# TheShadow29/VidSitu

Hardware: AMD Instinct MI355X
Metric: clips/s (10s@32x224x224) SlowFast+TxEnc fwd+bwd (higher is better)
Workload: dtype bf16

## Files before the change

include/vidsitu_hip.h:

```cpp
#ifndef VIDSITU_HIP_H
#define VIDSITU_HIP_H

#include <stddef.h>
#include <stdint.h>

#ifdef __cplusplus
extern "C" {
#endif

typedef enum vs_status {
  VS_OK = 0,
  VS_ERR_BAD_ARG = -1,
  VS_ERR_UNSUPPORTED = -2,
  VS_ERR_WORKSPACE = -3,
  VS_ERR_LAUNCH = -4
} vs_status;

#define VS_CONV_AFFINE 1
#define VS_CONV_RESIDUAL 2
#define VS_CONV_RELU 4
#define VS_CONV_STATS 8
#define VS_CONV_NAIVE 16
#define VS_CONV_TILE(id) (((id) + 1) << 8)
#define VS_CONV_RING(ns) (((ns) & 7) << 16)
// ... 88 lines not shown
                     const vs_dgrad_epilogue* ep, void* workspace, size_t ws_bytes, void* stream);
int vs_weight_transpose(const void* w, void* wt, int Cout, int taps, int Cin, void* stream);
int vs_weight_transpose_batched(const void* src, void* dst, const int64_t* table, int n,
                                int64_t total, void* stream);
int vs_transpose_f32_batched(const float* src, float* dst, const int64_t* table, int n, int64_t total,
                             void* stream);
int vs_weight_transpose_tiled(const void* src, void* dst, const int64_t* table, const int64_t* tile_first,
                              int n, int64_t total_tiles, int elem_bytes, void* stream);

#define VS_WGRAD_NODEEP (1 << 12)
#define VS_WGRAD_FORCEDEEP (1 << 13)
size_t vs_conv_wgrad_workspace_bytes(const vs_conv_desc* d);
int vs_conv_wgrad(const void* dy, const void* x, float* dw, const vs_conv_desc* d,
                  void* workspace, size_t ws_bytes, void* stream);
typedef struct vs_wgrad_item {
  const void* dy;
  const void* x;
  float* dw;
  vs_conv_desc d;
} vs_wgrad_item;
int vs_conv_wgrad_group_ok(const vs_wgrad_item* items, int n);
size_t vs_conv_wgrad_group_workspace_bytes(const vs_wgrad_item* items, int n);
int vs_conv_wgrad_group(const vs_wgrad_item* items, int n, void* workspace, size_t ws_bytes, void* stream);
int vs_conv_wgrad_partial(const void* dy, const void* x, float* dw, const vs_conv_desc* d, void* slabs,
                          size_t slab_bytes, int* splits, void* stream);
int64_t vs_wgrad_reduce_blocks(int64_t elements);
int vs_wgrad_reduce(const float* slabs, float* dw, int64_t elements, int splits, void* stream);
int vs_wgrad_reduce_batched(const int64_t* table, int n_entries, int64_t total_blocks, void* stream);
int vs_wgrad_reduce_defer(int mode);
int vs_wgrad_reduce_flush(void);

int vs_bn_finalize(const float* partials, int nparts, double count, const float* gamma,
                   const float* beta, float* running_mean, float* running_var, float momentum,
                   float eps, float* scale, float* shift, float* mean, float* invstd, int C,
                   void* stream);
size_t vs_bn_finalize_workspace_bytes(void);
int vs_bn_finalize_ws(const float* partials, int nparts, double count, const float* gamma, const float* beta,
                      float* running_mean, float* running_var, float momentum, float eps, float* scale,
                      float* shift, float* mean, float* invstd, int C, void* workspace, size_t ws_bytes,
                      void* stream);
int vs_bn_partials_reduce(const float* partials, int nparts, float* out, int C, int G,
                          void* stream);
int vs_bn_apply(const void* y, const float* scale, const float* shift, const void* residual,
                void* out, int64_t rows, int C, int y_ld, int res_ld, int out_ld, int relu,
                void* stream);
int vs_bn_apply_mask(const void* y, const float* scale, const float* shift, const void* residual,
// ... 180 lines not shown
```

vidsitu_amd/_lib.py:

```python
import ctypes as C
import os
import subprocess

_HERE = os.path.dirname(os.path.abspath(__file__))
LIB_PATH = os.environ.get("VS_LIB_PATH") or os.path.join(_HERE, "libvidsitu_hip.so")
CSRC_DIR = os.path.join(_HERE, "csrc")

VS_CONV_AFFINE = 1
VS_CONV_RESIDUAL = 2
VS_CONV_RELU = 4
VS_CONV_STATS = 8
VS_CONV_NAIVE = 16


class ConvDesc(C.Structure):

    _fields_ = [
        (n, C.c_int32)
        for n in (
            "N Ti Hi Wi Cin To Ho Wo Cout kT kH kW sT sH sW pT pH pW x_ld y_ld res_ld flags"
        ).split()
    ]


# ... 27 lines not shown
    "vs_conv_fwd": (_i, [_p, _p, _p, _dp, _p, _p, _p, _p, _p, _sz, _p]),
    "vs_conv_stats_rows": (_i, [_dp]),
    "vs_conv_workspace_bytes": (_sz, [_dp, _i]),
    "vs_conv_plan": (_i, [_dp, _i, _p]),
    "vs_conv_aol_ok": (_i, [_dp]),
    "vs_conv_fwd_aol": (_i, [_p, _p, _p, _dp, _p, _p, _p, _p]),
    "vs_conv_wgrad_aol_ok": (_i, [_dp]),
    "vs_conv_wgrad_aol": (_i, [_p, _p, _p, _dp, _p, _p, _p, _sz, _p]),
    "vs_conv_fwd_bc_fusable": (_i, [_dp, _i]),
    "vs_conv_fwd_bc": (_i, [_p, _p, _dp, _p, _p, _p, _i, _p, _p, _p, _i, _p, _i, _i, _p]),
    "vs_conv_dgrad": (_i, [_p, _p, _p, _dp, _p, _p, _sz, _p]),
    "vs_conv_dgrad_bnstats_rows": (_i, [_dp]),
    "vs_conv_dgrad_bnstats": (_i, [_p, _p, _p, _dp, _p, _p, _i, _p, _p, _p, _p, _p, _p, _p, _sz, _p]),
    "vs_conv_dgrad_ex": (_i, [_p, _p, _p, _dp, C.POINTER(DgradEpilogue), _p, _sz, _p]),
    "vs_weight_transpose": (_i, [_p, _p, _i, _i, _i, _p]),
    "vs_weight_transpose_batched": (_i, [_p, _p, _p, _i, _i64, _p]),
    "vs_transpose_f32_batched": (_i, [_p, _p, _p, _i, _i64, _p]),
    "vs_weight_transpose_tiled": (_i, [_p, _p, _p, _p, _i, _i64, _i, _p]),
    "vs_conv_wgrad_workspace_bytes": (_sz, [_dp]),
    "vs_conv_wgrad": (_i, [_p, _p, _p, _dp, _p, _sz, _p]),
    "vs_conv_wgrad_group_ok": (_i, [C.POINTER(WgradItem), _i]),
    "vs_conv_wgrad_group_workspace_bytes": (_sz, [C.POINTER(WgradItem), _i]),
    "vs_conv_wgrad_group": (_i, [C.POINTER(WgradItem), _i, _p, _sz, _p]),
    "vs_conv_wgrad_partial": (_i, [_p, _p, _p, _dp, _p, _sz, C.POINTER(C.c_int), _p]),
    "vs_wgrad_reduce_blocks": (_i64, [_i64]),
    "vs_wgrad_reduce": (_i, [_p, _p, _i64, _i, _p]),
    "vs_wgrad_reduce_batched": (_i, [_p, _i, _i64, _p]),
    "vs_wgrad_reduce_defer": (_i, [_i]),
    "vs_wgrad_reduce_flush": (_i, []),
    "vs_bn_finalize": (_i, [_p, _i, _d, _p, _p, _p, _p, _f, _f, _p, _p, _p, _p, _i, _p]),
    "vs_bn_finalize_workspace_bytes": (_sz, []),
    "vs_bn_finalize_ws": (_i, [_p, _i, _d, _p, _p, _p, _p, _f, _f, _p, _p, _p, _p, _i, _p, _sz, _p]),
    "vs_bn_bwd_finalize_ws": (_i, [_p, _i, _p, _p, _i, _p, _sz, _p]),
    "vs_bn_partials_reduce": (_i, [_p, _i, _p, _i, _i, _p]),
    "vs_bn_apply": (_i, [_p, _p, _p, _p, _p, _i64, _i, _i, _i, _i, _i, _p]),
    "vs_bn_apply_mask": (_i, [_p, _p, _p, _p, _p, _p, _i64, _i, _i, _i, _i, _p]),
    "vs_bn_apply2": (_i, [_p, _p, _p, _p, _p, _p, _p, _p, _i64, _i, _i, _i, _i, _p]),
    "vs_bn_bwd_reduce": (_i, [_p, _p, _p, _p, _p, _p, _p, _p, _i64, _i, _i, _i, _i, _i, _p]),
    "vs_bn_bwd_reduce_rows": (_i, [_i64, _i]),
    "vs_bn_bwd_finalize": (_i, [_p, _i, _p, _p, _i, _p]),
    "vs_bn_bwd_apply": (
        _i,
        [_p, _p, _p, _p, _p, _p, _p, _p, _p, _p, _p, _i64, _i, _i, _i, _i, _i, _i, _i, _p],
    ),
    "vs_bn_bwd_apply2": (_i, [_p] * 16 + [_i64, _i, _i, _i, _i, _i, _i, _p]),
    "vs_residual_add_f32": (_i, [_p, _p, _p, _p, _p, _i64, _i, _i, _i, _i, _i, _i, _p]),
# ... 121 lines not shown
```

vidsitu_amd/csrc/conv_wgrad.hip:

```cpp
#include <stdlib.h>

#include "common.h"

#include <mutex>
#include <type_traits>
#include "glue_bodies.h"

typedef __attribute__((ext_vector_type(4))) short s16x4;
typedef __attribute__((address_space(3))) s16x4 lds_s16x4;

struct WgradP {
  const uint16_t* dy;
  const uint16_t* x;
  float* out;
  int P;
  int Cout, Kp, Cin, x_ld, dy_ld;
  int To, Ho, Wo, Ti, Hi, Wi;
  int kT, kH, kW, sT, sH, sW, pT, pH, pW;
  int tilesM, tilesN, S, rows_per_split;
  unsigned x_bytes, dy_bytes;
  int xcd_order;
  int dbg;
  const float* in_scale;
  const float* in_shift;
};

#define WG_OOB 0x80000000u

#define WG_ROWTAB 1024

__device__ __forceinline__ int wg_swz_chunk(int row) {
  return ((row & 3) << 1) | (((row >> 3) & 1) << 3);
}

template <int BM, int BN, int WM, int WN, int MODE>
__global__ __launch_bounds__(256) void conv_wgrad_kernel(WgradP p) {
  extern __shared__ __attribute__((aligned(16))) char smem[];
  constexpr int TM = BM / WM, TN = BN / WN;
  constexpr int MR = TM / 16, NR = TN / 16;
  constexpr int CM = BM / 8, CN = BN / 8;
  constexpr int RPM = 256 / CM, RPN = 256 / CN;
  constexpr int IM = (64 + RPM - 1) / RPM, IN = (64 + RPN - 1) / RPN;
  constexpr int IMG = 64 * 256;
  constexpr int STAGE = 2 * IMG;
  static_assert(WM * WN == 4, "4 waves");

  const int tid = threadIdx.x;
  int bid = blockIdx.x;
  if (p.xcd_order) {
    const int nwg = gridDim.x, q = nwg >> 3, r = nwg & 7, xcd = blockIdx.x & 7;
    bid = (xcd < r ? xcd * (q + 1) : r * (q + 1) + (xcd - r) * q) + (blockIdx.x >> 3);
  }
  const int ntile = p.tilesM * p.tilesN;
  const int s = bid / ntile;
  bid -= s * ntile;
  const int tn = bid % p.tilesN, tm = bid / p.tilesN;
  const int m0 = tm * BM, n0 = tn * BN;
  const int pbeg = s * p.rows_per_split;
  const int pend = min(p.P, pbeg + p.rows_per_split);

  int4* rowtab = (int4*)(smem + 2 * STAGE);

  const int ccm = tid % CM, rm = tid / CM;
  const int ccn = tid % CN, rn = tid / CN;
  const bool mcol_ok = (m0 + ccm * 8) < p.Cout;
  const int ncol = n0 + ccn * 8;
  const bool ncol_ok = ncol < p.Kp;
  int dt = 0, dh = 0, dw = 0, c0 = 0;
  if (MODE == 1 && ncol_ok) {
    const int tap = ncol / p.Cin;
    c0 = ncol - tap * p.Cin;
    dw = tap % p.kW;
    const int t2 = tap / p.kW;
    dh = t2 % p.kH;
// ... 137 lines not shown
      gload(chunk0 + (st + 1) * 64, chunk0);
      __builtin_amdgcn_sched_barrier(0);
      compute(cur);
      __builtin_amdgcn_sched_barrier(0);
      sstore(cur ^ 1);
      __syncthreads();
    }
    compute((nsteps - 1) & 1);
    __syncthreads();
  }

  float* dst = p.out + (long long)s * p.Cout * p.Kp;
#pragma unroll
  for (int a = 0; a < MR; ++a)
#pragma unroll
    for (int b = 0; b < NR; ++b) {
      const int col = n0 + wn * TN + b * 16 + li;
#pragma unroll
      for (int r = 0; r < 4; ++r) {
        const int row = m0 + wm * TM + a * 16 + g * 4 + r;
        if (row < p.Cout && col < p.Kp) dst[(long long)row * p.Kp + col] = acc[a][b][r];
      }
    }
}

template <int BM, int BN, int WM, int WN, int MODE, int NS, bool AOL = false, int ROWS = 64>
__device__ __forceinline__ void conv_wgrad_ring_body(const WgradP& p, const int blk, const int nblk) {
  static_assert(!AOL || MODE == 0, "apply on load: pointwise launches");
  static_assert(ROWS == 64, "stage depth (the half-depth variant of round 4 was measured slower and removed)");
  extern __shared__ __attribute__((aligned(16))) char smem[];
  constexpr int TM = BM / WM, TN = BN / WN;
  constexpr int MR = TM / 16, NR = TN / 16;
  constexpr int CM = BM / 8, CN = BN / 8;
  constexpr int IMG = ROWS * 256;
  constexpr int STAGE = 2 * IMG;
  constexpr int D = NS - 1;
  constexpr int RG = ROWS / 16;
  constexpr int L = 2 * RG;
  constexpr int SPC = WG_ROWTAB / ROWS;
  static_assert(WM * WN == 4, "4 waves");
  static_assert((D - 1) * L <= 63, "vmcnt range");

  const int tid = threadIdx.x;
  int bid = blk;
  if (p.xcd_order) {
    const int nwg = nblk, q = nwg >> 3, r = nwg & 7, xcd = blk & 7;
// ... 504 lines not shown
  if (g.mode[j] == 0) conv_wgrad_deep_body<0, true>(g.p[j], b - lo, cnt);
  else conv_wgrad_deep_body<1, true>(g.p[j], b - lo, cnt);
}

struct WgReduceGroupP {
  int n;
  long long first[WGG_MAX + 1];
  const float* slabs[WGG_MAX];
  float* dw[WGG_MAX];
  long long len[WGG_MAX];
  int S[WGG_MAX];
};

__global__ __launch_bounds__(256) void wgrad_reduce_group_kernel(WgReduceGroupP g) {
  __shared__ float4 part[16][17];
  const long long b = blockIdx.x;
  int e = 0;
#pragma unroll
  for (int i = 1; i < WGG_MAX; ++i)
    if (i < g.n && b >= g.first[i]) e = i;
  wgrad_reduce_body(g.slabs[e], g.dw[e], g.len[e], g.S[e], part, b - g.first[e], threadIdx.x);
}

__global__ __launch_bounds__(256) void wgrad_reduce_kernel(const float* slabs, float* dw,
                                                          long long n, int S) {
  __shared__ float4 part[16][17];
  wgrad_reduce_body(slabs, dw, n, S, part, blockIdx.x, threadIdx.x);
}

namespace {
struct PendingState {
  int mode = 0;
  bool have = false;
  VsPendingReduce r{};
};
thread_local PendingState g_pending;

static void pending_launch(const VsPendingReduce& r) {
  const long long grid = wgrad_reduce_vblocks(r.n, r.S);
  hipLaunchKernelGGL(wgrad_reduce_kernel, dim3((unsigned)grid), dim3(256), 0, r.st, r.slabs, r.dw, r.n, r.S);
}
}

static void pending_flush() {
  if (g_pending.have) {
    g_pending.have = false;
    pending_launch(g_pending.r);
  }
}

static bool pending_stash(const float* slabs, float* dw, long long n, int S, hipStream_t st) {
  if (g_pending.mode != 1) return false;
  pending_flush();
  g_pending.r = VsPendingReduce{slabs, dw, n, S, st};
  g_pending.have = true;
  return true;
}

bool vs_pending_reduce_take(hipStream_t st, VsPendingReduce* out) {
  if (!g_pending.have || g_pending.r.st != st) return false;
  *out = g_pending.r;
  g_pending.have = false;
  return true;
}

extern "C" int vs_wgrad_reduce_defer(int mode) {
  VS_CHECK_ARG(mode >= 0 && mode <= 2, "mode 0 (off), 1 (defer), 2 (suspend)");
  if (mode == 0) pending_flush();
  g_pending.mode = mode;
  VS_CHECK_LAUNCH();
  return VS_OK;
}

extern "C" int vs_wgrad_reduce_flush(void) {
  pending_flush();
  VS_CHECK_LAUNCH();
  return VS_OK;
}

__global__ __launch_bounds__(256) void wgrad_reduce_batched_kernel(const long long* __restrict__ table, int nent) {
  __shared__ float4 part[16][17];
  const long long b = blockIdx.x;
  int lo = 0, hi = nent - 1;
  while (lo < hi) {
    const int mid = (lo + hi + 1) >> 1;
    if (table[mid * 5 + 4] <= b) lo = mid; else hi = mid - 1;
// ... 387 lines not shown

extern "C" size_t vs_conv_wgrad_group_workspace_bytes(const vs_wgrad_item* items, int n) {
  if (items == nullptr) return 0;
  WgCfg cfg[WGG_MAX];
  size_t off[WGG_MAX], tot = 0;
  int order[WGG_MAX];
  if (!wgg_plan(items, n, cfg, off, &tot, order)) return 0;
  return tot;
}

extern "C" int vs_conv_wgrad_group(const vs_wgrad_item* items, int n, void* workspace, size_t ws_bytes, void* stream) {
  VS_CHECK_ARG(items != nullptr && n >= 1 && n <= WGG_MAX, "1 .. 20 items");
  WgCfg cfg[WGG_MAX];
  size_t off[WGG_MAX], tot = 0;
  int order[WGG_MAX];
  if (!wgg_plan(items, n, cfg, off, &tot, order)) {
    vs_set_error("vs_conv_wgrad_group: an item is outside the deep-pipeline kernel's envelope (ask vs_conv_wgrad_group_ok)");
    return VS_ERR_UNSUPPORTED;
  }
  if (tot > 0 && (workspace == nullptr || ws_bytes < tot)) {
    vs_set_error("vs_conv_wgrad_group: workspace too small (%zu < %zu)", ws_bytes, tot);
    return VS_ERR_WORKSPACE;
  }
  if (g_pending.have) pending_flush();
  WgGroupP g;
  WgReduceGroupP r;
  g.n = n;
  r.n = 0;
  r.first[0] = 0;
  int first = 0;
  for (int a = 0; a < n; ++a) {
    const int j = order[a];
    const vs_wgrad_item& t = items[j];
    VS_CHECK_ARG(t.dy && t.x && t.dw, "null tensor");
    const vs_conv_desc* d = &t.d;
    float* out = cfg[j].S > 1 ? (float*)((char*)workspace + off[j]) : t.dw;
    const int rc = wg_fill_params(g.p[a], t.dy, t.x, out, d, cfg[j]);
    if (rc) return rc;
    const bool dense = (d->kT * d->kH * d->kW == 1) && d->sT == 1 && d->sH == 1 && d->sW == 1 && d->pT == 0 &&
                       d->pH == 0 && d->pW == 0;
    g.mode[a] = dense ? 0 : 1;
    g.first[a] = first;
    g.count[a] = cfg[j].tilesM * cfg[j].tilesN * cfg[j].S;
    first += g.count[a];
    if (cfg[j].S > 1) {
      const int e = r.n++;
      r.slabs[e] = out;
// ... 47 lines not shown
        for (int i = 0; i < cnt[x]; ++i) fprintf(stderr, " [slot %u p %u s %u t %u]", g.jobtab[x][i] >> 23, (g.jobtab[x][i] >> 18) & 31, (g.jobtab[x][i] >> 12) & 63, g.jobtab[x][i] & 4095);
        fprintf(stderr, "\n");
      }
      for (int a = 0; a < n; ++a) fprintf(stderr, "problem %d: tiles %d x %d S %d rps %d count %d\n", a, g.p[a].tilesM, g.p[a].tilesN, g.p[a].S, g.p[a].rows_per_split, g.count[a]);
#endif
      g.jobs = 1;
      grid = 8 * mx;
    }
  }
  static std::once_flag gattr;
  std::call_once(gattr, [] {
    (void)hipFuncSetAttribute((const void*)conv_wgrad_deep_group_kernel, hipFuncAttributeMaxDynamicSharedMemorySize, 160 * 1024);
  });
  const size_t smem = (size_t)WGD_NU * WGD_UNIT + 2 * WGD_TAB * sizeof(int2);
  hipLaunchKernelGGL(conv_wgrad_deep_group_kernel, dim3(grid), dim3(512), smem, (hipStream_t)stream, g);
  VS_CHECK_LAUNCH();
  if (r.n > 0) {
    hipLaunchKernelGGL(wgrad_reduce_group_kernel, dim3((unsigned)r.first[r.n]), dim3(256), 0, (hipStream_t)stream, r);
    VS_CHECK_LAUNCH();
  }
  return VS_OK;
}

static int wgrad_impl(const void* dy, const void* x, float* dw, const vs_conv_desc* d, void* workspace,
                      size_t ws_bytes, void* stream, bool reduce_now, int* splits_out,
                      const float* in_scale = nullptr, const float* in_shift = nullptr) {
  VS_CHECK_ARG(d && dy && x && dw, "null argument");
  VS_CHECK_ARG(d->Cin % 8 == 0 && d->Cout % 8 == 0, "Cin and Cout must be multiples of 8");
  VS_CHECK_ARG(d->x_ld % 8 == 0 && d->y_ld % 8 == 0, "row pitches must be multiples of 8");
  VS_CHECK_ARG((long long)d->N * d->Ti * d->Hi * d->Wi < (1ll << 31), "too many positions");
  const WgCfg c = wg_pick(d);
  const size_t need = vs_conv_wgrad_workspace_bytes(d);
  if (need > 0 && (workspace == nullptr || ws_bytes < need)) {
    vs_set_error("vs_conv_wgrad: workspace too small (%zu < %zu)", ws_bytes, need);
    return VS_ERR_WORKSPACE;
  }
  if (g_pending.have && ((const void*)g_pending.r.slabs == workspace || g_pending.r.dw == dw)) pending_flush();
  if (in_scale && !wgrad_aol_plan_ok(d)) {
    vs_set_error("vs_conv_wgrad_aol: apply on load is not built for this weight gradient (ask vs_conv_wgrad_aol_ok)");
    return VS_ERR_UNSUPPORTED;
  }
  WgradP p;
  {
    const int rc = wg_fill_params(p, dy, x, c.S > 1 ? (float*)workspace : dw, d, c);
    if (rc) return rc;
  }
  p.in_scale = in_scale;
  p.in_shift = in_shift;
  {
    static const int xo = [] { const char* e = getenv("VS_WGRAD_XCD"); return e ? atoi(e) : 1; }();
    p.xcd_order = xo && (c.tilesM * c.tilesN <= 32 || xo == 2 || (c.S % 8 == 0 && c.tilesM * c.tilesN <= 64));
    static const int dbg = [] { const char* e = getenv("VS_WGRAD_DBG"); return e ? atoi(e) : 0; }();
    p.dbg = dbg;
  }
  p.rows_per_split = c.rows_per_split;
  const bool dense = (d->kT * d->kH * d->kW == 1) && d->sT == 1 && d->sH == 1 && d->sW == 1 &&
                     d->pT == 0 && d->pH == 0 && d->pW == 0;
  const int mode = dense ? 0 : 1;
  hipStream_t st = (hipStream_t)stream;
  const int fring = (d->flags >> 16) & 7;
  int ring = fring == 1 ? 0 : (fring >= 2 ? (fring > 3 ? 3 : fring) : (c.bm == 128 ? 2 : 0));
  if (d->kT * d->kH * d->kW > 31) ring = 0;
  int rc;
  if (c.deep) {
    static std::once_flag dattr;
    std::call_once(dattr, [] {
      (void)hipFuncSetAttribute((const void*)conv_wgrad_deep_kernel<0, false>, hipFuncAttributeMaxDynamicSharedMemorySize, 160 * 1024);
      (void)hipFuncSetAttribute((const void*)conv_wgrad_deep_kernel<1, false>, hipFuncAttributeMaxDynamicSharedMemorySize, 160 * 1024);
      (void)hipFuncSetAttribute((const void*)conv_wgrad_deep_kernel<0, true>, hipFuncAttributeMaxDynamicSharedMemorySize, 160 * 1024);
      (void)hipFuncSetAttribute((const void*)conv_wgrad_deep_kernel<1, true>, hipFuncAttributeMaxDynamicSharedMemorySize, 160 * 1024);
    });
    static const int stag = [] { const char* e = getenv("VS_WGRAD_DEEP_STAG"); return e ? atoi(e) : 1; }();
    if (in_scale) {
      vs_set_error("vs_conv_wgrad_aol: not built for the deep-pipeline plan");
      return VS_ERR_UNSUPPORTED;
    }
    const size_t smem = (size_t)WGD_NU * WGD_UNIT + 2 * WGD_TAB * sizeof(int2);
// ... 50 lines not shown
```

vidsitu_amd/ops.py:

```python
import ctypes as C

import torch

from . import _lib
from ._lib import (
    VS_CONV_AFFINE,
    VS_CONV_NAIVE,
    VS_CONV_RELU,
    VS_CONV_RESIDUAL,
    VS_CONV_STATS,
    ConvDesc,
)

BF16 = torch.bfloat16


def _stream():
    return C.c_void_p(torch.cuda.current_stream().cuda_stream)


def _ptr(t):
    if t is None:
        return None
    if not t.is_cuda:
# ... 489 lines not shown
            raise _lib.VsError("conv_wgrad out must be fp32 with [Cout][taps][Cin] memory")
        arr[i].dy, arr[i].x, arr[i].dw = dy.data_ptr(), x.data_ptr(), out.data_ptr()
        arr[i].d = make_desc(x.shape, act_ld(x), dy.shape, act_ld(dy), k, s, p, 0)
        _ptr(dy), _ptr(x), _ptr(out)
    return arr


def conv_wgrad_group_ok(items):
    if not 1 <= len(items) <= WGRAD_GROUP_MAX:
        return False
    return bool(_lib.load().vs_conv_wgrad_group_ok(_wgrad_items(items), len(items)))


def conv_wgrad_group(items):
    if _WHATIF_WGRAD:
        return
    arr = _wgrad_items(items)
    need = int(_lib.load().vs_conv_wgrad_group_workspace_bytes(arr, len(items)))
    ws = _workspace(need, items[0][0].device, "wgrad") if need else None
    _lib.call("vs_conv_wgrad_group", arr, len(items), _ptr(ws), C.c_size_t(ws.numel() if ws is not None else 0),
              _stream())


def conv_wgrad(dy, x, k, s, p, out=None, ring=0, batch=None, tile=None, slots=0, deep=True):
    cout, cin = dy.shape[1], x.shape[1]
    if out is None:
        out = torch.empty((cout, *k, cin), dtype=torch.float32, device=x.device).permute(0, 4, 1, 2, 3)
    elif not out.permute(0, 2, 3, 4, 1).is_contiguous() or out.dtype != torch.float32:
        raise _lib.VsError("conv_wgrad out must be fp32 with [Cout][taps][Cin] memory")
    if batch is not None:
        return batch.wgrad(dy, x, k, s, p, out, ring)
    if _WHATIF_WGRAD:
        return out
    flags = ((ring & 7) << 16) | (((tile + 1) << 8) if tile is not None else 0) | (((slots // 8) & 0xff) << 24)
    if not deep:
        flags |= 1 << 12
    elif deep == "force":
        flags |= 1 << 13
    d = make_desc(x.shape, act_ld(x), dy.shape, act_ld(dy), k, s, p, flags)
    need = _lib.load().vs_conv_wgrad_workspace_bytes(C.byref(d))
    ws = _workspace(need, x.device, "wgrad") if need else None
    _lib.call("vs_conv_wgrad", _ptr(dy), _ptr(x), _ptr(out), C.byref(d), _ptr(ws),
              C.c_size_t(ws.numel() if ws is not None else 0), _stream())
    return out


# ... 791 lines not shown
```

vidsitu_amd/trunk.py:

```python
import contextlib
import os

import torch
from torch import nn

from . import ops

STAGE_DEPTH = {50: (3, 4, 6, 3), 101: (3, 4, 23, 3), "tiny": (1, 0, 0, 1), "mini": (1, 1, 1, 1)}
TEMPORAL_KERNEL_BASIS = {
    "c2d": [[[1]], [[1]], [[1]], [[1]], [[1]]],
    "i3d": [[[5]], [[3]], [[3, 1]], [[3, 1]], [[1, 3]]],
    "slow": [[[1]], [[1]], [[1]], [[3]], [[3]]],
    "slowfast": [[[1], [5]], [[1], [3]], [[1], [3]], [[3], [3]], [[3], [3]]],
}
POOL1 = {
    "c2d": [[2, 1, 1]],
    "i3d": [[2, 1, 1]],
    "slow": [[1, 1, 1]],
    "slowfast": [[1, 1, 1], [1, 1, 1]],
}


class Conv3dP(nn.Module):

# ... 481 lines not shown
            yb, aff = _Unit.fwd(b2.b, b2.b_bn, a, True, train=True, saved=saved, no_apply=True)
            z = _Unit.fwd(b2.c, b2.c_bn, yb, True, residual=sc, out=out, train=True, saved=saved, x_affine=aff)
            if self.has_sc and saved is not None and len(saved) >= 4:
                saved[-1]["sc_rec"] = saved[-4]
            return z
        if not train and self._bc_fusable(a):
            (sb, hb), (s_c, h_c) = b2.b_bn.fold, b2.c_bn.fold
            return ops.conv_fwd_bc(a, b2.b.w_bf16, b2.b.k, b2.b.s, b2.b.p, sb, hb, b2.c.w_bf16, s_c, h_c,
                                   residual=sc, relu=True, out=out)
        b = _Unit.fwd(b2.b, b2.b_bn, a, True, train=train, saved=saved)
        if ResBlock.residual_fp32 and not train:
            branch = _Unit.fwd(b2.c, b2.c_bn, b, False, train=False)
            res = sc if self.has_sc else getattr(x, "_vs_f32", x)
            z, z32 = ops.residual_add_f32(branch, res, relu=True, out16=out)
            z._vs_f32 = z32
            return z
        z = _Unit.fwd(b2.c, b2.c_bn, b, True, residual=sc, out=out, train=train, saved=saved)
        if self.has_sc and train and saved is not None and len(saved) >= 4:
            saved[-1]["sc_rec"] = saved[-4]
        return z

    def bwd(self, saved, dout, chain=False, carry=None):
        rc, rb, ra = saved.pop(), saved.pop(), saved.pop()
        sink = [] if self._wgrad_grouped(rc, rb, ra, saved[-1] if (self.has_sc and saved) else None, dout) else None
        res = self._bwd_units(saved, dout, chain, rc, rb, ra, sink)
        if sink:
            items = [(dy, x, c.k, c.s, c.p, c.weight.grad) for dy, x, c in sink]
            if carry is None:
                ops.conv_wgrad_group(items)
            else:
                carry["items"] += items
                carry["blocks"] += 1
                if carry["blocks"] >= ResBlock.group_span or len(carry["items"]) + 4 > ops.WGRAD_GROUP_MAX:
                    ResBlock.flush_wgrads(carry)
        return res

    @staticmethod
    def flush_wgrads(carry):
        if carry and carry["items"]:
            items = carry["items"]
            ops.conv_wgrad_group(items)
        if carry:
            carry["items"], carry["blocks"] = [], 0


    group_span = int(os.environ.get("VS_WGRAD_GROUP_SPAN", "3"))

    group_wgrads = os.environ.get("VS_WGRAD_GROUP", "1") != "0"
    group_max_positions = int(os.environ.get("VS_WGRAD_GROUP_MAXP", "1000000000"))
    group_min_channels = int(os.environ.get("VS_WGRAD_GROUP_MINC", "128"))

    def _wgrad_grouped(self, rc, rb, ra, rsc, dout):
        if (not ResBlock.group_wgrads or not dout.is_cuda or _Unit.wgrad_batch is not None or _Unit.split_wgrad_reduce
                or ResBlock.aol):
            return False
        recs = [r for r in (rc, rb, ra, rsc) if r is not None]
        key = ("wgg",) + tuple(tuple(r["y"].shape) for r in recs)
        hit = self.__dict__.setdefault("_bc_ok", {}).get(key)
        if hit is None:
            hit = True
            items = []
            for r in recs:
                c, y, x = r["conv"], r["y"], r["x"]
                if (c.is_stem or c.cin_pad != c.cin or c.bias is not None or r.get("x_affine") is not None
                        or c.cout < ResBlock.group_min_channels or not isinstance(x, torch.Tensor)
                        or not getattr(c.weight, "_vs_direct_grad", True)):
                    hit = False
                    break
                items.append((y, x, c.k, c.s, c.p, torch.empty(0)))
            if hit:
                hit = min(ops.act_rows(r["y"]) for r in recs) <= ResBlock.group_max_positions
            if hit:
                probe = [(y, x, k, s_, p, torch.empty((y.shape[1], *k, x.shape[1]), dtype=torch.float32,
                                                      device=y.device).permute(0, 4, 1, 2, 3)) for y, x, k, s_, p, _ in items]
                hit = ops.conv_wgrad_group_ok(probe)
            self._bc_ok[key] = hit
        return hit

    def _bwd_units(self, saved, dout, chain, rc, rb, ra, sink):
        cbits = rc.get("zbits")
        dy_sc = None
        if (self.has_sc and cbits is not None and ResBlock.fuse_sc_bwd and dout.is_cuda and saved
                and rc["conv"].bias is None and saved[-1]["conv"].bias is None and ops.bn_apply2_ok(rc["y"].shape[1])):
            rsc = saved[-1]
            units = []
            for r in (rc, rsc):
                bn = r["bn"]
                if bn.weight.grad is None:
                    bn.weight.grad = torch.zeros_like(bn.weight)
                if bn.bias.grad is None:
                    bn.bias.grad = torch.zeros_like(bn.bias)
                ops.bn_bwd_sums(dout, r["y"], r["mean"], r["invstd"], cbits, bn.weight.grad, bn.bias.grad,
                                partial=r.pop("bwd_partial", None))
                units.append((r["y"], r["mean"], r["invstd"], bn.weight, bn.weight.grad, bn.bias.grad))
            dy_c, dy_sc = ops.bn_bwd_apply2(dout, cbits, units[0], units[1])
            db, g = _Unit.bwd(rc, dout, producer=rb, dy_ready=dy_c, wgrad_sink=sink)
        else:
            db, g = _Unit.bwd(rc, dout, want_dres=cbits is None, producer=rb, wgrad_sink=sink)
# ... 158 lines not shown
            dx = ops.conv_dgrad(dtheta, self.conv_theta.wt(), tuple(x.shape), self.K1, self.S1, self.P0,
                                residual=dpool)
            return ops.bn_apply(dx, self._vec(c, 1.0, dev), self._vec(c, 0.0, dev), dres, relu=False)
        dx = ops.conv_dgrad(dtheta, self.conv_theta.wt(), tuple(x.shape), self.K1, self.S1, self.P0, residual=dres)
        dx = ops.conv_dgrad(dphi, self.conv_phi.wt(), tuple(x.shape), self.K1, self.S1, self.P0, residual=dx)
        return ops.conv_dgrad(dg, self.conv_g.wt(), tuple(x.shape), self.K1, self.S1, self.P0, residual=dx)


class ResStage(nn.Module):
    def __init__(self, cins, couts, cinners, tks, strides, nblocks, nblk_tk, eps, mom, zero_final,
                 nl_inds=None, nl_pool=None, nl_inst="dot_product"):
        super().__init__()
        self.num_pathways = len(cins)
        self.num_blocks = list(nblocks)
        self.couts = list(couts)
        self.nl_inds = [list(v) for v in nl_inds] if nl_inds is not None else [[] for _ in cins]
        for p in range(self.num_pathways):
            for i in self.nl_inds[p]:
                self.add_module(f"pathway{p}_nonlocal{i}",
                                Nonlocal(couts[p], couts[p] // 2, nl_pool[p], nl_inst, eps, mom))
            n = nblocks[p]
            tk_list = (tks[p] * n)[: nblk_tk[p]] + [1] * (n - nblk_tk[p])
            for i in range(n):
                self.add_module(
                    f"pathway{p}_res{i}",
                    ResBlock(cins[p] if i == 0 else couts[p], couts[p], cinners[p], tk_list[i],
                             strides[p] if i == 0 else 1, eps, mom, zero_final))

    def blocks(self, p):
        out = []
        for i in range(self.num_blocks[p]):
            out.append(getattr(self, f"pathway{p}_res{i}"))
            if i in self.nl_inds[p]:
                out.append(getattr(self, f"pathway{p}_nonlocal{i}"))
        return out


class PathwayPool(nn.Module):

    def __init__(self, kt):
        super().__init__()
        self.kt = kt

    def forward(self, x):
        return x if self.kt == 1 else ops.maxpool_t(x, self.kt)[0]


class _TrunkFn(torch.autograd.Function):

    @staticmethod
# ... 464 lines not shown
```

Before: 728.1.

## Group fast-pathway weight-gradient convs into one tile/ring kernel launch

Adds a grouped launcher that runs several non-deep weight-gradient convolutions (tile or ring bodies) in a single kernel, dispatching each block to its item by prefix offsets. It is used for the SlowFast fast pathway, whose small-channel convs were previously excluded from grouping. The pending split-reduce queue becomes a multi-entry queue that flushes only on conflicting buffers and batches queued reductions into grouped reduce launches. This targets per-launch overhead and tail underutilization, at the cost of double-buffered workspaces, more host bookkeeping, and a changed grouping cache key.

```diff
diff --git a/include/vidsitu_hip.h b/include/vidsitu_hip.h
--- a/include/vidsitu_hip.h
+++ b/include/vidsitu_hip.h
@@ -134,6 +134,9 @@
 int vs_conv_wgrad_group_ok(const vs_wgrad_item* items, int n);
 size_t vs_conv_wgrad_group_workspace_bytes(const vs_wgrad_item* items, int n);
 int vs_conv_wgrad_group(const vs_wgrad_item* items, int n, void* workspace, size_t ws_bytes, void* stream);
+int vs_conv_wgrad_group_tile_ok(const vs_wgrad_item* items, int n);
+size_t vs_conv_wgrad_group_tile_workspace_bytes(const vs_wgrad_item* items, int n);
+int vs_conv_wgrad_group_tile(const vs_wgrad_item* items, int n, void* workspace, size_t ws_bytes, void* stream);
 int vs_conv_wgrad_partial(const void* dy, const void* x, float* dw, const vs_conv_desc* d, void* slabs,
                           size_t slab_bytes, int* splits, void* stream);
 int64_t vs_wgrad_reduce_blocks(int64_t elements);
diff --git a/vidsitu_amd/_lib.py b/vidsitu_amd/_lib.py
--- a/vidsitu_amd/_lib.py
+++ b/vidsitu_amd/_lib.py
@@ -73,6 +73,9 @@
     "vs_conv_wgrad_group_ok": (_i, [C.POINTER(WgradItem), _i]),
     "vs_conv_wgrad_group_workspace_bytes": (_sz, [C.POINTER(WgradItem), _i]),
     "vs_conv_wgrad_group": (_i, [C.POINTER(WgradItem), _i, _p, _sz, _p]),
+    "vs_conv_wgrad_group_tile_ok": (_i, [C.POINTER(WgradItem), _i]),
+    "vs_conv_wgrad_group_tile_workspace_bytes": (_sz, [C.POINTER(WgradItem), _i]),
+    "vs_conv_wgrad_group_tile": (_i, [C.POINTER(WgradItem), _i, _p, _sz, _p]),
     "vs_conv_wgrad_partial": (_i, [_p, _p, _p, _dp, _p, _sz, C.POINTER(C.c_int), _p]),
     "vs_wgrad_reduce_blocks": (_i64, [_i64]),
     "vs_wgrad_reduce": (_i, [_p, _p, _i64, _i, _p]),
diff --git a/vidsitu_amd/csrc/conv_wgrad.hip b/vidsitu_amd/csrc/conv_wgrad.hip
--- a/vidsitu_amd/csrc/conv_wgrad.hip
+++ b/vidsitu_amd/csrc/conv_wgrad.hip
@@ -34,7 +34,7 @@
 }
 
 template <int BM, int BN, int WM, int WN, int MODE>
-__global__ __launch_bounds__(256) void conv_wgrad_kernel(WgradP p) {
+__device__ __forceinline__ void conv_wgrad_tile_body(const WgradP& p, const int blk, const int nblk) {
   extern __shared__ __attribute__((aligned(16))) char smem[];
   constexpr int TM = BM / WM, TN = BN / WN;
   constexpr int MR = TM / 16, NR = TN / 16;
@@ -46,10 +46,10 @@
   static_assert(WM * WN == 4, "4 waves");
 
   const int tid = threadIdx.x;
-  int bid = blockIdx.x;
+  int bid = blk;
   if (p.xcd_order) {
-    const int nwg = gridDim.x, q = nwg >> 3, r = nwg & 7, xcd = blockIdx.x & 7;
-    bid = (xcd < r ? xcd * (q + 1) : r * (q + 1) + (xcd - r) * q) + (blockIdx.x >> 3);
+    const int nwg = nblk, q = nwg >> 3, r = nwg & 7, xcd = blk & 7;
+    bid = (xcd < r ? xcd * (q + 1) : r * (q + 1) + (xcd - r) * q) + (blk >> 3);
   }
   const int ntile = p.tilesM * p.tilesN;
   const int s = bid / ntile;
@@ -233,6 +233,11 @@
         if (row < p.Cout && col < p.Kp) dst[(long long)row * p.Kp + col] = acc[a][b][r];
       }
     }
+}
+
+template <int BM, int BN, int WM, int WN, int MODE>
+__global__ __launch_bounds__(256) void conv_wgrad_kernel(WgradP p) {
+  conv_wgrad_tile_body<BM, BN, WM, WN, MODE>(p, blockIdx.x, gridDim.x);
 }
 
 template <int BM, int BN, int WM, int WN, int MODE, int NS, bool AOL = false, int ROWS = 64>
@@ -783,17 +788,41 @@
   wgrad_reduce_body(g.slabs[e], g.dw[e], g.len[e], g.S[e], part, b - g.first[e], threadIdx.x);
 }
 
+#define WGT_MAX 20
+struct WgTileGroupP {
+  int n;
+  int first[WGT_MAX + 1];
+  int count[WGT_MAX];
+  WgradP p[WGT_MAX];
+};
+static_assert(sizeof(WgTileGroupP) <= 4096, "kernel arguments");
+
+template <int BM, int BN, int WM, int WN, int MODE, bool RING>
+__global__ __launch_bounds__(256) void conv_wgrad_tile_group_kernel(WgTileGroupP g) {
+  const int b = blockIdx.x;
+  int j = 0;
+#pragma unroll
+  for (int i = 1; i < WGT_MAX; ++i)
+    if (i < g.n && b >= g.first[i]) j = i;
+  j = __builtin_amdgcn_readfirstlane(j);
+  const int lo = g.first[j], cnt = g.count[j];
+  if (b - lo >= cnt) return;
+  if constexpr (RING) conv_wgrad_ring_body<BM, BN, WM, WN, MODE, 2>(g.p[j], b - lo, cnt);
+  else conv_wgrad_tile_body<BM, BN, WM, WN, MODE>(g.p[j], b - lo, cnt);
+}
+
 __global__ __launch_bounds__(256) void wgrad_reduce_kernel(const float* slabs, float* dw,
                                                           long long n, int S) {
   __shared__ float4 part[16][17];
   wgrad_reduce_body(slabs, dw, n, S, part, blockIdx.x, threadIdx.x);
 }
 
+#define WG_PENDING_MAX 32
 namespace {
 struct PendingState {
   int mode = 0;
-  bool have = false;
-  VsPendingReduce r{};
+  int n = 0;
+  VsPendingReduce q[WG_PENDING_MAX];
 };
 thread_local PendingState g_pending;
 
@@ -801,28 +830,84 @@
   const long long grid = wgrad_reduce_vblocks(r.n, r.S);
   hipLaunchKernelGGL(wgrad_reduce_kernel, dim3((unsigned)grid), dim3(256), 0, r.st, r.slabs, r.dw, r.n, r.S);
 }
+
+static void pending_launch_marked(const bool* take) {
+  bool done[WG_PENDING_MAX] = {};
+  for (int e = 0; e < g_pending.n; ++e) {
+    if (!take[e] || done[e]) continue;
+    const hipStream_t st = g_pending.q[e].st;
+    WgReduceGroupP r;
+    r.n = 0;
+    r.first[0] = 0;
+    int last = e;
+    for (int f = e; f < g_pending.n && r.n < WGG_MAX; ++f) {
+      if (!take[f] || done[f] || g_pending.q[f].st != st) continue;
+      const VsPendingReduce& x = g_pending.q[f];
+      r.slabs[r.n] = x.slabs;
+      r.dw[r.n] = x.dw;
+      r.len[r.n] = x.n;
+      r.S[r.n] = x.S;
+      r.first[r.n + 1] = r.first[r.n] + wgrad_reduce_vblocks(x.n, x.S);
+      ++r.n;
+      done[f] = true;
+      last = f;
+    }
+    if (r.n == 1) {
+      pending_launch(g_pending.q[last]);
+    } else {
+      for (int i = r.n + 1; i <= WGG_MAX; ++i) r.first[i] = r.first[r.n];
+      hipLaunchKernelGGL(wgrad_reduce_group_kernel, dim3((unsigned)r.first[r.n]), dim3(256), 0, st, r);
+    }
+  }
+  int k = 0;
+  for (int e = 0; e < g_pending.n; ++e)
+    if (!take[e]) g_pending.q[k++] = g_pending.q[e];
+  g_pending.n = k;
+}
 }
 
 static void pending_flush() {
-  if (g_pending.have) {
-    g_pending.have = false;
-    pending_launch(g_pending.r);
-  }
+  if (g_pending.n == 0) return;
+  bool take[WG_PENDING_MAX];
+  for (int e = 0; e < WG_PENDING_MAX; ++e) take[e] = true;
+  pending_launch_marked(take);
+}
+
+static void pending_flush_conflicts(const void* lo, size_t bytes, const float* dw) {
+  if (g_pending.n == 0) return;
+  bool take[WG_PENDING_MAX] = {}, any = false;
+  const char* a = (const char*)lo;
+  for (int e = 0; e < g_pending.n; ++e) {
+    const VsPendingReduce& x = g_pending.q[e];
+    const char* s0 = (const char*)x.slabs;
+    const char* s1 = s0 + (size_t)x.n * (size_t)x.S * sizeof(float);
+    take[e] = (a && bytes && s0 < a + bytes && a < s1) || (dw && x.dw == dw);
+    any |= take[e];
+  }
+  if (any) pending_launch_marked(take);
 }
 
 static bool pending_stash(const float* slabs, float* dw, long long n, int S, hipStream_t st) {
   if (g_pending.mode != 1) return false;
-  pending_flush();
-  g_pending.r = VsPendingReduce{slabs, dw, n, S, st};
-  g_pending.have = true;
+  pending_flush_conflicts(slabs, (size_t)n * (size_t)S * sizeof(float), dw);
+  if (g_pending.n == WG_PENDING_MAX) {
+    pending_launch(g_pending.q[0]);
+    for (int e = 1; e < g_pending.n; ++e) g_pending.q[e - 1] = g_pending.q[e];
+    --g_pending.n;
+  }
+  g_pending.q[g_pending.n++] = VsPendingReduce{slabs, dw, n, S, st};
   return true;
 }
 
 bool vs_pending_reduce_take(hipStream_t st, VsPendingReduce* out) {
-  if (!g_pending.have || g_pending.r.st != st) return false;
-  *out = g_pending.r;
-  g_pending.have = false;
-  return true;
+  for (int e = 0; e < g_pending.n; ++e) {
+    if (g_pending.q[e].st != st) continue;
+    *out = g_pending.q[e];
+    for (int f = e + 1; f < g_pending.n; ++f) g_pending.q[f - 1] = g_pending.q[f];
+    --g_pending.n;
+    return true;
+  }
+  return false;
 }
 
 extern "C" int vs_wgrad_reduce_defer(int mode) {
@@ -1256,7 +1341,7 @@
     vs_set_error("vs_conv_wgrad_group: workspace too small (%zu < %zu)", ws_bytes, tot);
     return VS_ERR_WORKSPACE;
   }
-  if (g_pending.have) pending_flush();
+  pending_flush();
   WgGroupP g;
   WgReduceGroupP r;
   g.n = n;
@@ -1350,6 +1435,176 @@
   return VS_OK;
 }
 
+static void wg_order_flags(WgradP& p, const WgCfg& c) {
+  static const int xo = [] { const char* e = getenv("VS_WGRAD_XCD"); return e ? atoi(e) : 1; }();
+  p.xcd_order = xo && (c.tilesM * c.tilesN <= 32 || xo == 2 || (c.S % 8 == 0 && c.tilesM * c.tilesN <= 64));
+  static const int dbg = [] { const char* e = getenv("VS_WGRAD_DBG"); return e ? atoi(e) : 0; }();
+  p.dbg = dbg;
+}
+
+struct WgtPlan {
+  WgCfg c;
+  int mode, ring;
+  size_t off;
+};
+
+static bool wgt_item_plan(const vs_conv_desc* d, WgtPlan* w) {
+  if (d->N < 1 || d->Cin < 8 || d->Cout < 8 || d->Cin % 8 || d->Cout % 8 || d->x_ld % 8 || d->y_ld % 8) return false;
+  if (d->flags != 0 || d->kT < 1 || d->kH < 1 || d->kW < 1) return false;
+  const long long P = (long long)d->N * d->To * d->Ho * d->Wo;
+  const long long xb = (long long)d->N * d->Ti * d->Hi * d->Wi * d->x_ld * 2;
+  const long long db = P * d->y_ld * 2;
+  if (P < 1 || (long long)d->N * d->Ti * d->Hi * d->Wi >= (1ll << 31) || xb >= (1ll << 31) || db >= (1ll << 31))
+    return false;
+  const WgCfg c = wg_pick(d);
+  if (c.deep) return false;
+  const int taps = d->kT * d->kH * d->kW;
+  const bool dense = taps == 1 && d->sT == 1 && d->sH == 1 && d->sW == 1 && d->pT == 0 && d->pH == 0 && d->pW == 0;
+  const int ring = (c.bm == 128 && taps <= 31) ? 2 : 0;
+  if (c.bm == 128 && ring == 0) return false;
+  if ((long long)c.tilesM * c.tilesN * c.S > 65535) return false;
+  w->c = c;
+  w->mode = dense ? 0 : 1;
+  w->ring = ring;
+  return true;
+}
+
+static bool wgt_plan(const vs_wgrad_item* it, int n, WgtPlan* w, size_t* total) {
+  if (it == nullptr || n < 1 || n > WGT_MAX) return false;
+  size_t off = 0;
+  for (int j = 0; j < n; ++j) {
+    if (!wgt_item_plan(&it[j].d, &w[j])) return false;
+    w[j].off = off;
+    if (w[j].c.S > 1) {
+      const size_t b = (size_t)w[j].c.S * it[j].d.Cout * it[j].d.kT * it[j].d.kH * it[j].d.kW * it[j].d.Cin * sizeof(float);
+      off += (b + 255) & ~(size_t)255;
+    }
+  }
+  *total = off;
+  return true;
+}
+
+extern "C" int vs_conv_wgrad_group_tile_ok(const vs_wgrad_item* items, int n) {
+  WgtPlan w[WGT_MAX];
+  size_t tot = 0;
+  return wgt_plan(items, n, w, &tot) ? 1 : 0;
+}
+
+extern "C" size_t vs_conv_wgrad_group_tile_workspace_bytes(const vs_wgrad_item* items, int n) {
+  WgtPlan w[WGT_MAX];
+  size_t tot = 0;
+  return wgt_plan(items, n, w, &tot) ? tot : 0;
+}
+
+template <int BM, int BN, int WM, int WN>
+static void wgt_launch(const WgTileGroupP& g, int grid, int mode, hipStream_t st) {
+  if constexpr (BM == 128) {
+    static std::once_flag once;
+    std::call_once(once, [] {
+      (void)hipFuncSetAttribute((const void*)conv_wgrad_tile_group_kernel<BM, BN, WM, WN, 0, true>,
+                                hipFuncAttributeMaxDynamicSharedMemorySize, 160 * 1024);
+      (void)hipFuncSetAttribute((const void*)conv_wgrad_tile_group_kernel<BM, BN, WM, WN, 1, true>,
+                                hipFuncAttributeMaxDynamicSharedMemorySize, 160 * 1024);
+    });
+    const size_t smem = (size_t)2 * 2 * 64 * 256 + (mode ? 2 * WG_ROWTAB * sizeof(int2) : 0);
+    if (mode == 0)
+      hipLaunchKernelGGL((conv_wgrad_tile_group_kernel<BM, BN, WM, WN, 0, true>), dim3(grid), dim3(256), smem, st, g);
+    else
+      hipLaunchKernelGGL((conv_wgrad_tile_group_kernel<BM, BN, WM, WN, 1, true>), dim3(grid), dim3(256), smem, st, g);
+  } else {
+    static std::once_flag once;
+    std::call_once(once, [] {
+      (void)hipFuncSetAttribute((const void*)conv_wgrad_tile_group_kernel<BM, BN, WM, WN, 0, false>,
+                                hipFuncAttributeMaxDynamicSharedMemorySize, 160 * 1024);
+      (void)hipFuncSetAttribute((const void*)conv_wgrad_tile_group_kernel<BM, BN, WM, WN, 1, false>,
+                                hipFuncAttributeMaxDynamicSharedMemorySize, 160 * 1024);
+    });
+    const size_t smem = (size_t)2 * 2 * 64 * 256 + (mode ? WG_ROWTAB * sizeof(int4) : 0);
+    if (mode == 0)
+      hipLaunchKernelGGL((conv_wgrad_tile_group_kernel<BM, BN, WM, WN, 0, false>), dim3(grid), dim3(256), smem, st, g);
+    else
+      hipLaunchKernelGGL((conv_wgrad_tile_group_kernel<BM, BN, WM, WN, 1, false>), dim3(grid), dim3(256), smem, st, g);
+  }
+}
+
+extern "C" int vs_conv_wgrad_group_tile(const vs_wgrad_item* items, int n, void* workspace, size_t ws_bytes,
+                                        void* stream) {
+  VS_CHECK_ARG(items != nullptr && n >= 1 && n <= WGT_MAX, "1 .. 20 items");
+  WgtPlan w[WGT_MAX];
+  size_t tot = 0;
+  if (!wgt_plan(items, n, w, &tot)) {
+    vs_set_error("vs_conv_wgrad_group_tile: an item is outside the tile / ring bodies' envelope (ask vs_conv_wgrad_group_tile_ok)");
+    return VS_ERR_UNSUPPORTED;
+  }
+  if (tot > 0 && (workspace == nullptr || ws_bytes < tot)) {
+    vs_set_error("vs_conv_wgrad_group_tile: workspace too small (%zu < %zu)", ws_bytes, tot);
+    return VS_ERR_WORKSPACE;
+  }
+  for (int j = 0; j < n; ++j) VS_CHECK_ARG(items[j].dy && items[j].x && items[j].dw, "null tensor");
+  pending_flush_conflicts(workspace, tot, nullptr);
+  for (int j = 0; j < n; ++j) pending_flush_conflicts(nullptr, 0, items[j].dw);
+  hipStream_t st = (hipStream_t)stream;
+  bool done[WGT_MAX] = {};
+  for (int a = 0; a < n; ++a) {
+    if (done[a]) continue;
+    int mem[WGT_MAX], m = 0;
+    for (int j = a; j < n; ++j)
+      if (!done[j] && w[j].c.bm == w[a].c.bm && w[j].c.bn == w[a].c.bn && w[j].mode == w[a].mode && w[j].ring == w[a].ring) {
+        mem[m++] = j;
+        done[j] = true;
+      }
+    for (int x = 1; x < m; ++x)
+      for (int y = x; y > 0 && w[mem[y]].c.rows_per_split > w[mem[y - 1]].c.rows_per_split; --y) {
+        const int t = mem[y];
+        mem[y] = mem[y - 1];
+        mem[y - 1] = t;
+      }
+    WgTileGroupP g;
+    g.n = m;
+    int first = 0, grid = 0;
+    for (int k = 0; k < WGT_MAX; ++k) {
+      if (k < m) {
+        const int j = mem[k];
+        const vs_wgrad_item& t = items[j];
+        float* out = w[j].c.S > 1 ? (float*)((char*)workspace + w[j].off) : t.dw;
+        const int rc = wg_fill_params(g.p[k], t.dy, t.x, out, &t.d, w[j].c);
+        if (rc) return rc;
+        wg_order_flags(g.p[k], w[j].c);
+        g.first[k] = first;
+        g.count[k] = w[j].c.tilesM * w[j].c.tilesN * w[j].c.S;
+        grid = first + g.count[k];
+        first = (grid + 7) & ~7;
+      } else {
+        g.p[k] = g.p[0];
+        g.first[k] = first;
+        g.count[k] = 0;
+      }
+    }
+    g.first[WGT_MAX] = first;
+    const WgCfg& c = w[a].c;
+    if (c.bm == 128 && c.bn == 128) wgt_launch<128, 128, 2, 2>(g, grid, w[a].mode, st);
+    else if (c.bm == 128) wgt_launch<128, 64, 2, 2>(g, grid, w[a].mode, st);
+    else if (c.bm == 64 && c.bn == 128) wgt_launch<64, 128, 2, 2>(g, grid, w[a].mode, st);
+    else if (c.bm == 64) wgt_launch<64, 64, 2, 2>(g, grid, w[a].mode, st);
+    else if (c.bm == 32 && c.bn == 128) wgt_launch<32, 128, 1, 4>(g, grid, w[a].mode, st);
+    else if (c.bm == 32) wgt_launch<32, 64, 1, 4>(g, grid, w[a].mode, st);
+    else if (c.bn == 128) wgt_launch<16, 128, 1, 4>(g, grid, w[a].mode, st);
+    else wgt_launch<16, 64, 1, 4>(g, grid, w[a].mode, st);
+    VS_CHECK_LAUNCH();
+  }
+  for (int j = 0; j < n; ++j) {
+    if (w[j].c.S <= 1) continue;
+    const float* slabs = (const float*)((const char*)workspace + w[j].off);
+    const long long ne = (long long)items[j].d.Cout * items[j].d.kT * items[j].d.kH * items[j].d.kW * items[j].d.Cin;
+    if (!pending_stash(slabs, items[j].dw, ne, w[j].c.S, st)) {
+      hipLaunchKernelGGL(wgrad_reduce_kernel, dim3((unsigned)wgrad_reduce_vblocks(ne, w[j].c.S)), dim3(256), 0, st, slabs,
+                         items[j].dw, ne, w[j].c.S);
+      VS_CHECK_LAUNCH();
+    }
+  }
+  return VS_OK;
+}
+
 static int wgrad_impl(const void* dy, const void* x, float* dw, const vs_conv_desc* d, void* workspace,
                       size_t ws_bytes, void* stream, bool reduce_now, int* splits_out,
                       const float* in_scale = nullptr, const float* in_shift = nullptr) {
@@ -1363,7 +1618,7 @@
     vs_set_error("vs_conv_wgrad: workspace too small (%zu < %zu)", ws_bytes, need);
     return VS_ERR_WORKSPACE;
   }
-  if (g_pending.have && ((const void*)g_pending.r.slabs == workspace || g_pending.r.dw == dw)) pending_flush();
+  pending_flush_conflicts(workspace, ws_bytes, dw);
   if (in_scale && !wgrad_aol_plan_ok(d)) {
     vs_set_error("vs_conv_wgrad_aol: apply on load is not built for this weight gradient (ask vs_conv_wgrad_aol_ok)");
     return VS_ERR_UNSUPPORTED;
@@ -1375,12 +1630,7 @@
   }
   p.in_scale = in_scale;
   p.in_shift = in_shift;
-  {
-    static const int xo = [] { const char* e = getenv("VS_WGRAD_XCD"); return e ? atoi(e) : 1; }();
-    p.xcd_order = xo && (c.tilesM * c.tilesN <= 32 || xo == 2 || (c.S % 8 == 0 && c.tilesM * c.tilesN <= 64));
-    static const int dbg = [] { const char* e = getenv("VS_WGRAD_DBG"); return e ? atoi(e) : 0; }();
-    p.dbg = dbg;
-  }
+  wg_order_flags(p, c);
   p.rows_per_split = c.rows_per_split;
   const bool dense = (d->kT * d->kH * d->kW == 1) && d->sT == 1 && d->sH == 1 && d->sW == 1 &&
                      d->pT == 0 && d->pH == 0 && d->pW == 0;
diff --git a/vidsitu_amd/ops.py b/vidsitu_amd/ops.py
--- a/vidsitu_amd/ops.py
+++ b/vidsitu_amd/ops.py
@@ -535,6 +535,35 @@
               _stream())
 
 
+WGRAD_GROUP_TILE_MAX = 20
+
+
+def conv_wgrad_group_tile_ok(items):
+    if not 1 <= len(items) <= WGRAD_GROUP_TILE_MAX:
+        return False
+    return bool(_lib.load().vs_conv_wgrad_group_tile_ok(_wgrad_items(items), len(items)))
+
+
+def conv_wgrad_group_tile(items):
+    if _WHATIF_WGRAD:
+        return
+    arr = _wgrad_items(items)
+    need = int(_lib.load().vs_conv_wgrad_group_tile_workspace_bytes(arr, len(items)))
+    ws = None
+    if need:
+        dev = items[0][0].device
+        key = (dev.index, torch.cuda.current_stream().cuda_stream)
+        turn = _tile_ws_turn.get(key, 0)
+        _tile_ws_turn[key] = turn ^ 1
+        pair = [_workspace(need, dev, "wgrad_tile0"), _workspace(need, dev, "wgrad_tile1")]
+        ws = pair[turn]
+    _lib.call("vs_conv_wgrad_group_tile", arr, len(items), _ptr(ws), C.c_size_t(ws.numel() if ws is not None else 0),
+              _stream())
+
+
+_tile_ws_turn = {}
+
+
 def conv_wgrad(dy, x, k, s, p, out=None, ring=0, batch=None, tile=None, slots=0, deep=True):
     cout, cin = dy.shape[1], x.shape[1]
     if out is None:
diff --git a/vidsitu_amd/trunk.py b/vidsitu_amd/trunk.py
--- a/vidsitu_amd/trunk.py
+++ b/vidsitu_amd/trunk.py
@@ -527,24 +527,33 @@
 
     def bwd(self, saved, dout, chain=False, carry=None):
         rc, rb, ra = saved.pop(), saved.pop(), saved.pop()
-        sink = [] if self._wgrad_grouped(rc, rb, ra, saved[-1] if (self.has_sc and saved) else None, dout) else None
+        path = self._wgrad_grouped(rc, rb, ra, saved[-1] if (self.has_sc and saved) else None, dout)
+        sink = [] if path else None
         res = self._bwd_units(saved, dout, chain, rc, rb, ra, sink)
         if sink:
             items = [(dy, x, c.k, c.s, c.p, c.weight.grad) for dy, x, c in sink]
             if carry is None:
-                ops.conv_wgrad_group(items)
+                (ops.conv_wgrad_group if path == "deep" else ops.conv_wgrad_group_tile)(items)
             else:
-                carry["items"] += items
+                if carry["items"] and carry["items"][0][0] != path:
+                    ResBlock.flush_wgrads(carry)
+                carry["items"] += [(path,) + it for it in items]
                 carry["blocks"] += 1
-                if carry["blocks"] >= ResBlock.group_span or len(carry["items"]) + 4 > ops.WGRAD_GROUP_MAX:
+                span, cap = ((ResBlock.group_span, ops.WGRAD_GROUP_MAX) if path == "deep"
+                             else (ResBlock.group_tile_span, ops.WGRAD_GROUP_TILE_MAX))
+                if carry["blocks"] >= span or len(carry["items"]) + 4 > cap:
                     ResBlock.flush_wgrads(carry)
         return res
 
     @staticmethod
     def flush_wgrads(carry):
         if carry and carry["items"]:
-            items = carry["items"]
-            ops.conv_wgrad_group(items)
+            deep = [it[1:] for it in carry["items"] if it[0] == "deep"]
+            tile = [it[1:] for it in carry["items"] if it[0] == "tile"]
+            if deep:
+                ops.conv_wgrad_group(deep)
+            if tile:
+                ops.conv_wgrad_group_tile(tile)
         if carry:
             carry["items"], carry["blocks"] = [], 0
 
@@ -555,30 +564,36 @@
     group_max_positions = int(os.environ.get("VS_WGRAD_GROUP_MAXP", "1000000000"))
     group_min_channels = int(os.environ.get("VS_WGRAD_GROUP_MINC", "128"))
 
+    group_tile = os.environ.get("VS_WGRAD_GROUP_TILE", "1") != "0"
+    group_tile_span = int(os.environ.get("VS_WGRAD_GROUP_TILE_SPAN", "6"))
+    fast_pathway = False
+
     def _wgrad_grouped(self, rc, rb, ra, rsc, dout):
         if (not ResBlock.group_wgrads or not dout.is_cuda or _Unit.wgrad_batch is not None or _Unit.split_wgrad_reduce
                 or ResBlock.aol):
-            return False
+            return None
         recs = [r for r in (rc, rb, ra, rsc) if r is not None]
-        key = ("wgg",) + tuple(tuple(r["y"].shape) for r in recs)
-        hit = self.__dict__.setdefault("_bc_ok", {}).get(key)
-        if hit is None:
-            hit = True
+        key = ("wgg", ResBlock.group_tile) + tuple(tuple(r["y"].shape) for r in recs)
+        hit = self.__dict__.setdefault("_bc_ok", {}).get(key, False)
+        if hit is False:
+            hit = None
             items = []
             for r in recs:
                 c, y, x = r["conv"], r["y"], r["x"]
                 if (c.is_stem or c.cin_pad != c.cin or c.bias is not None or r.get("x_affine") is not None
-                        or c.cout < ResBlock.group_min_channels or not isinstance(x, torch.Tensor)
-                        or not getattr(c.weight, "_vs_direct_grad", True)):
-                    hit = False
+                        or not isinstance(x, torch.Tensor) or not getattr(c.weight, "_vs_direct_grad", True)):
+                    items = None
                     break
                 items.append((y, x, c.k, c.s, c.p, torch.empty(0)))
-            if hit:
-                hit = min(ops.act_rows(r["y"]) for r in recs) <= ResBlock.group_max_positions
-            if hit:
+            if items:
                 probe = [(y, x, k, s_, p, torch.empty((y.shape[1], *k, x.shape[1]), dtype=torch.float32,
                                                       device=y.device).permute(0, 4, 1, 2, 3)) for y, x, k, s_, p, _ in items]
-                hit = ops.conv_wgrad_group_ok(probe)
+                if (min(r["conv"].cout for r in recs) >= ResBlock.group_min_channels
+                        and min(ops.act_rows(r["y"]) for r in recs) <= ResBlock.group_max_positions
+                        and ops.conv_wgrad_group_ok(probe)):
+                    hit = "deep"
+                elif self.fast_pathway and ResBlock.group_tile and ops.conv_wgrad_group_tile_ok(probe):
+                    hit = "tile"
             self._bc_ok[key] = hit
         return hit
 
@@ -783,10 +798,10 @@
             n = nblocks[p]
             tk_list = (tks[p] * n)[: nblk_tk[p]] + [1] * (n - nblk_tk[p])
             for i in range(n):
-                self.add_module(
-                    f"pathway{p}_res{i}",
-                    ResBlock(cins[p] if i == 0 else couts[p], couts[p], cinners[p], tk_list[i],
-                             strides[p] if i == 0 else 1, eps, mom, zero_final))
+                blk = ResBlock(cins[p] if i == 0 else couts[p], couts[p], cinners[p], tk_list[i],
+                               strides[p] if i == 0 else 1, eps, mom, zero_final)
+                blk.fast_pathway = self.num_pathways > 1 and p == 1
+                self.add_module(f"pathway{p}_res{i}", blk)
 
     def blocks(self, p):
         out = []
```

Result: faster. 735.7 (median of 6 runs) (+1.0%).
